# nuclia/nucliadb

Hardware: AMD Instinct MI355X
Metric: queries/sec + recall@10 (768-dim cosine k-NN, HNSW M=30 ef=30 ef_upper=4 build_ef_upper=4, k=10) (higher is better)
Workload: dtype f32

## Files before the change

### nucliadb_amd/csrc/hnsw_device.h

```cpp
#pragma once
#include "device_common.h"
#include "kernels.h"

namespace nidx {

#define NIDX_POOL_CAP 512
#define NIDX_VIS_EMPTY 0xffffffffu
#define NIDX_DEFER_CAP 256

struct NbBuf {
    uint32_t addr[64];
    float ab[64];
    float xx[64];
};
struct SearchShared {
    uint64_t pool[NIDX_POOL_CAP];
    NbBuf nb[2];
    uint32_t eps[256];
    int ctrl[12];
};

template <int NJ>
struct QueryRegs {
    float4 qv[NJ];
    float qq;
    double sqrt_qq;
};

template <int NJ>
__device__ inline void load_query(QueryRegs<NJ> &q, const float *qrow, uint32_t dp, int lane, bool cosine) {
    float acc = 0.f;
#pragma unroll
    for (int j = 0; j < NJ; j++) {
        q.qv[j] = load_row_chunk(qrow, dp, j, lane);
        acc = fma4(q.qv[j], q.qv[j], acc);
    }
    q.qq = wave_butterfly_sum(acc);
    q.sqrt_qq = cosine ? sqrt((double)q.qq) : 0.0;
}

__device__ inline float score_from_sums(float ab, float xx, float qq, double sqrt_qq, bool cosine) {
    if (!cosine) return ab;
    double dab = (double)ab, dxx = (double)xx;
    double dist;
    if (dxx == 0.0 && (double)qq == 0.0) dist = 0.0;
    else if (dab == 0.0) dist = 1.0;
    else {
        double d = 1.0 - dab / (sqrt(dxx) * sqrt_qq);
        dist = d > 0.0 ? d : 0.0;
    }
    return 1.0f - (float)dist;
}

__device__ inline uint32_t nidx_tid() {
    const uint32_t nw = blockDim.x >> 6;
    const uint32_t t = threadIdx.x + ((blockIdx.x % nw) << 6);
    return t >= blockDim.x ? t - blockDim.x : t;
}

__device__ inline void vis_clear(uint32_t *vis, uint32_t cap) {
    for (uint32_t i = nidx_tid(); i < cap; i += blockDim.x) vis[i] = NIDX_VIS_EMPTY;
}
__device__ inline bool vis_insert(uint32_t *vis, uint32_t log2cap, uint32_t v) {
    const uint32_t mask = (1u << log2cap) - 1u;
    uint32_t h = (v * 2654435761u) >> (32 - log2cap);
    for (;;) {
        uint32_t old = atomicCAS(&vis[h], NIDX_VIS_EMPTY, v);
        if (old == NIDX_VIS_EMPTY) return true;
        if (old == v) return false;
        h = (h + 1) & mask;
    }
}

__device__ inline bool vis_contains(const uint32_t *vis, uint32_t log2cap, uint32_t v) {
    const uint32_t mask = (1u << log2cap) - 1u;
    uint32_t h = (v * 2654435761u) >> (32 - log2cap);
    for (;;) {
        const uint32_t cur = vis[h];
        if (cur == NIDX_VIS_EMPTY) return false;
        if (cur == v) return true;
        h = (h + 1) & mask;
    }
}

__device__ inline uint64_t wave_max_u64(uint64_t v) { return wave_extreme_u64<true>(v); }
__device__ inline uint64_t wave_min_u64(uint64_t v) { return wave_extreme_u64<false>(v); }
__device__ inline uint64_t pool_peek(const uint64_t *pool, int pool_len, int lane) {
    uint64_t best = NIDX_EMPTY_KEY;
    for (int i = lane; i < pool_len; i += 64) {
        uint64_t v = pool[i];
        best = v > best ? v : best;
    }
    return wave_max_u64(best);
}
__device__ inline uint64_t pool_pop(uint64_t *pool, int &pool_len, int lane) {
    if (pool_len == 0) return NIDX_EMPTY_KEY;
    uint64_t best = NIDX_EMPTY_KEY;
    for (int i = lane; i < pool_len; i += 64) {
        uint64_t v = pool[i];
        best = v > best ? v : best;
    }
    best = wave_max_u64(best);
    int idx = 0x7fffffff;
    for (int i = lane; i < pool_len; i += 64)
        if (pool[i] == best && i < idx) idx = i;
    idx = wave_min_i32(idx);
    uint64_t last = pool[pool_len - 1];
    if (lane == 0) pool[idx] = last;
    pool_len--;
    return best;
}
__device__ inline void pool_prune(uint64_t *pool, int &pool_len, float ws, int lane) {
    int out = 0;
    for (int base = 0; base < pool_len; base += 64) {
        int i = base + lane;
        uint64_t v = i < pool_len ? pool[i] : NIDX_EMPTY_KEY;
        bool keep = i < pool_len && !(rank_key_score(v) < ws);
        unsigned long long m = __ballot(keep);
        int pos = out + __popcll(m & ((1ull << lane) - 1ull));
        if (keep) pool[pos] = v;
        out += __popcll(m);
    }
    pool_len = out;
}

template <int NL>
struct CandSet {
    uint64_t unexp[NL];
    __device__ inline void init() {
#pragma unroll
        for (int i = 0; i < NL; i++) unexp[i] = 0;
    }
    __device__ inline void insert(WaveTopK<NL> &res, uint64_t nk, int cap, int lane, uint64_t &out_key, bool &out_unexp) {
        uint64_t d = nk, dflag = 1;
#pragma unroll
        for (int i = 0; i < NL; i++) {
            if (d != NIDX_EMPTY_KEY) {
                const int pos = __popcll(__ballot(res.l[i].key > d));
                if (pos < 64) {
                    const uint64_t last = lane_bcast_u64(res.l[i].key, 63);
                    const uint64_t lastflag = unexp[i] >> 63;
                    const uint64_t up = wave_shr1_u64(res.l[i].key);
                    if (lane > pos) res.l[i].key = up;
                    if (lane == pos) res.l[i].key = d;
                    const uint64_t low = unexp[i] & ((1ull << pos) - 1ull);
                    const uint64_t high = pos < 63 ? ((unexp[i] >> pos) << (pos + 1)) : 0ull;
                    unexp[i] = low | (dflag << pos) | high;
                    d = last;
                    dflag = lastflag;
                }
            }
        }
        res.len++;
        out_key = NIDX_EMPTY_KEY;
        out_unexp = false;
        if (res.len > cap) {
            if (cap >= 64 * NL) {
                out_key = d;
                out_unexp = dflag != 0;
            }
#pragma unroll
            for (int i = 0; i < NL; i++)
                if ((cap >> 6) == i) {
                    out_key = lane_bcast_u64(res.l[i].key, cap & 63);
                    out_unexp = ((unexp[i] >> (cap & 63)) & 1ull) != 0;
                    if (lane == (cap & 63)) res.l[i].key = NIDX_EMPTY_KEY;
                    unexp[i] &= ~(1ull << (cap & 63));
                }
            res.len = cap;
        }
    }
    __device__ inline uint64_t peek(const WaveTopK<NL> &res) const {
#pragma unroll
        for (int i = 0; i < NL; i++)
            if (unexp[i]) return lane_bcast_u64(res.l[i].key, __builtin_ctzll(unexp[i]));
        return NIDX_EMPTY_KEY;
    }
    __device__ inline void peek2_except(const WaveTopK<NL> &res, uint64_t skip, uint64_t &a, uint64_t &b) const {
        a = b = NIDX_EMPTY_KEY;
        int found = 0;
#pragma unroll
        for (int i = 0; i < NL; i++) {
            uint64_t m = unexp[i];
            while (m && found < 2) {
                const uint64_t key = lane_bcast_u64(res.l[i].key, __builtin_ctzll(m));
                m &= m - 1ull;
                if (key == skip) continue;
                if (found == 0) a = key;
                else b = key;
                found++;
            }
        }
    }
    __device__ inline uint64_t pop(const WaveTopK<NL> &res) {
#pragma unroll
        for (int i = 0; i < NL; i++)
            if (unexp[i]) {
                const int r = __builtin_ctzll(unexp[i]);
                unexp[i] &= unexp[i] - 1ull;
                return lane_bcast_u64(res.l[i].key, r);
            }
        return NIDX_EMPTY_KEY;
    }
};

struct SearchCounters {
    uint32_t evals, expansions, visited, flags, edge_hits;
    uint64_t cyc_ctl, cyc_eval, cyc_ins;
};

template <int NJ, int EVR>
__device__ inline void eval_row_group(const SegDev &seg, const QueryRegs<NJ> &q, NbBuf &nb, int base, int n, bool cosine, int lane) {
    float4 row[EVR][NJ];
#pragma unroll
    for (int i = 0; i < EVR; i++) {
        if (base + i < n) {
            const float *r = seg.vectors + (size_t)nb.addr[base + i] * seg.dp;
#pragma unroll
            for (int j = 0; j < NJ; j++) row[i][j] = load_row_chunk(r, seg.dp, j, lane);
        } else {
#pragma unroll
            for (int j = 0; j < NJ; j++) row[i][j] = make_float4(0.f, 0.f, 0.f, 0.f);
        }
    }
    constexpr int NV_COS = 2 * EVR <= 2 ? 2 : (2 * EVR <= 4 ? 4 : 8);
    constexpr int NV_DOT = EVR <= 1 ? 1 : (EVR <= 2 ? 2 : 4);
    if (cosine) {
        float v[NV_COS];
#pragma unroll
        for (int i = 0; i < NV_COS; i++) v[i] = 0.f;
#pragma unroll
        for (int i = 0; i < EVR; i++) {
            float ab = 0.f, xx = 0.f;
#pragma unroll
            for (int j = 0; j < NJ; j++) {
                ab = fma4(row[i][j], q.qv[j], ab);
                xx = fma4(row[i][j], row[i][j], xx);
            }
            v[2 * i] = ab;
            v[2 * i + 1] = xx;
        }
        float r = QReduce<NV_COS>::run(v, lane);
        int which = QReduce<NV_COS>::query_of_lane(lane);
        if ((lane & QReduce<NV_COS>::group_mask()) == 0) {
            int i = which >> 1;
            if (i < EVR && base + i < n) {
                if ((which & 1) == 0) nb.ab[base + i] = r;
                else nb.xx[base + i] = r;
            }
        }
    } else {
        float v[NV_DOT];
#pragma unroll
        for (int i = 0; i < NV_DOT; i++) v[i] = 0.f;
#pragma unroll
        for (int i = 0; i < EVR; i++) {
            float ab = 0.f;
#pragma unroll
            for (int j = 0; j < NJ; j++) ab = fma4(row[i][j], q.qv[j], ab);
            v[i] = ab;
        }
        float r = QReduce<NV_DOT>::run(v, lane);
        int which = QReduce<NV_DOT>::query_of_lane(lane);
        if ((lane & QReduce<NV_DOT>::group_mask()) == 0 && which < EVR && base + which < n) nb.ab[base + which] = r;
    }
}

template <int NJ, int EVR>
__device__ inline void eval_neighbours(const SegDev &seg, const QueryRegs<NJ> &q, NbBuf &nb, int n, bool cosine) {
    const int lane = threadIdx.x & 63;
    const int wave = nidx_tid() >> 6;
    const int nwaves = blockDim.x >> 6;
    for (int base = wave * EVR; base < n; base += nwaves * EVR) eval_row_group<NJ, EVR>(seg, q, nb, base, n, cosine, lane);
}

template <int NJ, int EVR>
__device__ inline void eval_neighbours_dynamic(const SegDev &seg, const QueryRegs<NJ> &q, NbBuf &nb, int n, bool cosine, int *next_row) {
    const int lane = threadIdx.x & 63;
    for (;;) {
        int base = 0;
        if (lane == 0) base = atomicAdd(next_row, EVR);
        base = __builtin_amdgcn_readfirstlane(base);
        if (base >= n) break;
        eval_row_group<NJ, EVR>(seg, q, nb, base, n, cosine, lane);
    }
}

#define NIDX_CMD_EVAL 0
#define NIDX_CMD_CLEAR 1
#define NIDX_CMD_EXIT 2
__device__ inline void split_post(SearchShared &sh, int op, int p, int n, int lane) {
    if (lane == 0) {
        sh.ctrl[0] = op | (p << 2) | (n << 3);
        sh.ctrl[3] = 0;
    }
    lds_barrier();
}
__device__ inline void split_close() { lds_barrier(); }
__device__ inline uint32_t load_edge_word(const GraphDev &g, uint32_t node, int layer, int lane, uint32_t &deg) {
    uint32_t w = 0;
    if (layer == 0) {
        w = g.l0[(size_t)node * NIDX_L0_STRIDE + lane];
    } else {
        uint32_t base = g.upper_base[node];
        if (base != 0xffffffffu && lane < NIDX_UP_STRIDE) w = g.upper[((size_t)base + (layer - 1)) * NIDX_UP_STRIDE + lane];
    }
    deg = lane_bcast_u32(w, 0);
    return w;
}

template <int NJ, int EVR>
__device__ inline void split_worker_loop(const SegDev &seg, const QueryRegs<NJ> &q, SearchShared &sh, uint32_t *vis, uint32_t vis_cap, bool cosine) {
    for (;;) {
        lds_barrier();
        const int cmd = __builtin_amdgcn_readfirstlane(sh.ctrl[0]);
        const int op = cmd & 3;
        if (op == NIDX_CMD_EVAL) eval_neighbours_dynamic<NJ, EVR>(seg, q, sh.nb[(cmd >> 2) & 1], cmd >> 3, cosine, &sh.ctrl[3]);
        else if (op == NIDX_CMD_CLEAR) vis_clear(vis, vis_cap);
        lds_barrier();
        if (op == NIDX_CMD_EXIT) return;
    }
}

#define NIDX_PARK_SLOTS 4
#define NIDX_EPS_BARE 0
#define NIDX_EPS_PARKED 1
#define NIDX_EPS_CARRIED 2
template <int NJ, int EFL, int EVR, bool SPLIT = false>
__device__ inline void layer_search_block(const SegDev &seg, const GraphDev &g, int layer, int k,
                                          const QueryRegs<NJ> &q, SearchShared &sh, uint32_t *vis, uint32_t vis_log2,
                                          WaveTopK<EFL> &res, SearchCounters &st, int ep_mode = NIDX_EPS_BARE) {
    const int lane = threadIdx.x & 63;
    const bool ctl = SPLIT ? true : (nidx_tid() >> 6) == 0;
    const bool cosine = seg.similarity == 1;
    const uint32_t vis_cap = 1u << vis_log2;
    const bool carried = ep_mode == NIDX_EPS_CARRIED;
    int pool_len = 0;
    uint32_t vis_count = 0;

    if constexpr (SPLIT) {
        split_post(sh, NIDX_CMD_CLEAR, 0, 0, lane);
        vis_clear(vis, vis_cap);
        split_close();
    } else {
        vis_clear(vis, vis_cap);
        __syncthreads();
    }
    int n_new = sh.ctrl[2];
    if (n_new > k) k = n_new < 64 * EFL ? n_new : 64 * EFL;
    CandSet<EFL> cand;
    cand.init();
    const int n_eps = carried ? 0 : n_new;
    uint32_t ptag = 0xffffffffu, pbase = 0xffffffffu;
    uint32_t pt0 = 0xffffffffu, pt1 = 0xffffffffu, pt2 = 0xffffffffu, pt3 = 0xffffffffu;
    int n_park = 0;
    if (ep_mode != NIDX_EPS_BARE && n_new <= 64) n_park = n_new < NIDX_PARK_SLOTS ? n_new : NIDX_PARK_SLOTS;
    if (carried && ctl) {
#pragma unroll
        for (int i = 0; i < EFL; i++) {
            const int left = res.len - 64 * i;
            cand.unexp[i] = left >= 64 ? ~0ull : (left > 0 ? (1ull << left) - 1ull : 0ull);
            if (lane < left) vis_insert(vis, vis_log2, rank_key_addr(res.mine(i)));
        }
        st.evals += n_new;
        vis_count += n_new;
        if (lane < n_park) ptag = rank_key_addr(res.mine(0));
    }
    if (ctl && !carried) {
        res.init();
        if (lane < n_new) {
            uint32_t ep = sh.eps[lane];
            vis_insert(vis, vis_log2, ep);
            sh.nb[0].addr[lane] = ep;
            if (lane < n_park) ptag = ep;
        }
    }
    if (layer >= 1 && ptag != 0xffffffffu) pbase = g.upper_base[ptag];
    int ep_done = 0;
    while (ep_done < n_eps) {
        int chunk = n_eps - ep_done < 64 ? n_eps - ep_done : 64;
        if (ctl && ep_done > 0 && lane < chunk) {
            uint32_t ep = sh.eps[ep_done + lane];
            vis_insert(vis, vis_log2, ep);
            sh.nb[0].addr[lane] = ep;
        }
        if constexpr (SPLIT) {
            split_post(sh, NIDX_CMD_EVAL, 0, chunk, lane);
            split_close();
        } else {
            __syncthreads();
            eval_neighbours<NJ, EVR>(seg, q, sh.nb[0], chunk, cosine);
            __syncthreads();
        }
        if (ctl) {
            float s = lane < chunk ? score_from_sums(sh.nb[0].ab[lane], sh.nb[0].xx[lane], q.qq, q.sqrt_qq, cosine) : 0.f;
            uint32_t addr = sh.nb[0].addr[lane];
            for (int j = 0; j < chunk; j++) {
                uint64_t ek;
                bool eu;
                cand.insert(res, rank_key(lane_bcast_f32(s, j), lane_bcast_u32(addr, j)), 64 * EFL, lane, ek, eu);
            }
            st.evals += chunk;
            vis_count += chunk;
        }
        ep_done += chunk;
    }
    if (ctl && n_park > 0) {
        pt0 = lane_bcast_u32(ptag, 0);
        pt1 = lane_bcast_u32(ptag, 1);
        pt2 = lane_bcast_u32(ptag, 2);
        pt3 = lane_bcast_u32(ptag, 3);
        uint32_t w[NIDX_PARK_SLOTS];
#pragma unroll
        for (int r = 0; r < NIDX_PARK_SLOTS; r++) {
            w[r] = 0;
            if (r < n_park) {
                const uint32_t node = lane_bcast_u32(ptag, r), b = lane_bcast_u32(pbase, r);
                if (layer == 0) w[r] = g.l0[(size_t)node * NIDX_L0_STRIDE + lane];
                else if (b != 0xffffffffu && lane < NIDX_UP_STRIDE) w[r] = g.upper[((size_t)b + (layer - 1)) * NIDX_UP_STRIDE + lane];
            }
        }
#pragma unroll
        for (int r = 0; r < NIDX_PARK_SLOTS; r++)
            if (r < n_park) sh.eps[r * 64 + lane] = w[r];
    }

    uint32_t pw0 = 0, pw1 = 0, tg0 = 0xffffffffu, tg1 = 0xffffffffu;
    uint32_t edge_hits = 0;
    auto prepare = [&](uint64_t ck, NbBuf &dst) -> int {
        uint32_t deg;
        const uint32_t node = rank_key_addr(ck);
        uint32_t w;
        const int slot = node == pt0 ? 0 : (node == pt1 ? 1 : (node == pt2 ? 2 : (node == pt3 ? 3 : -1)));
        if (slot >= 0) {
            w = sh.eps[slot * 64 + lane];
            deg = lane_bcast_u32(w, 0);
            edge_hits++;
        } else if (node == tg0) {
            w = pw0;
            deg = lane_bcast_u32(w, 0);
            edge_hits++;
        } else if (node == tg1) {
            w = pw1;
            deg = lane_bcast_u32(w, 0);
            edge_hits++;
        } else {
            w = load_edge_word(g, node, layer, lane, deg);
        }
        const bool fresh = lane >= 1 && lane <= (int)deg && !vis_contains(vis, vis_log2, w);
        const unsigned long long m = __ballot(fresh);
        if (fresh) dst.addr[__popcll(m & ((1ull << lane) - 1ull))] = w;
        return __popcll(m);
    };
    int p = 0;
    uint64_t cur = NIDX_EMPTY_KEY;
    int cont = 0, n_cur_reg = 0;
    if (ctl) {
        const uint64_t t_a = clock64();
        int n0 = 0;
        cur = cand.pop(res);
        if (cur != NIDX_EMPTY_KEY && !(rank_key_score(cur) < res.worst_score())) {
            cont = 1;
            n0 = prepare(cur, sh.nb[0]);
        }
        n_cur_reg = n0;
        if (!SPLIT && lane == 0) {
            sh.ctrl[0] = cont;
            sh.ctrl[6] = n0;
            sh.ctrl[3] = 0;
        }
        st.cyc_ctl += clock64() - t_a;
    }
    if constexpr (SPLIT) {
        if (cont) {
            split_post(sh, NIDX_CMD_EVAL, 0, n_cur_reg, lane);
            split_close();
        }
    } else {
        lds_barrier();
        cont = sh.ctrl[0];
        if (cont) {
            eval_neighbours_dynamic<NJ, EVR>(seg, q, sh.nb[0], sh.ctrl[6], cosine, &sh.ctrl[3]);
            lds_barrier();
        }
    }
    if (cont) {
        for (;;) {
            NbBuf &nb_cur = sh.nb[p], &nb_next = sh.nb[p ^ 1];
            const int n_cur = SPLIT ? n_cur_reg : sh.ctrl[6 + p];
            float s = 0.f;
            uint32_t addr = 0;
            unsigned long long todo = 0;
            uint64_t nxt = NIDX_EMPTY_KEY;
            bool overflow = false;
            int n_next_reg = 0, redo_reg = 0;
            const uint64_t t_a = clock64();
            if (ctl) {
                const bool mine = lane < n_cur;
                addr = nb_cur.addr[lane];
                bool ins = mine && vis_insert(vis, vis_log2, addr);
                unsigned long long failed = __ballot(mine && !ins);
                while (failed) {
                    const int f = __ffsll((long long)failed) - 1;
                    failed &= failed - 1;
                    const unsigned long long same = __ballot(mine && addr == lane_bcast_u32(addr, f));
                    if ((same >> lane) & 1ull) ins = lane == __ffsll((long long)same) - 1;
                }
                todo = __ballot(ins);
                const int n_valid = __popcll(todo);
                st.expansions++;
                st.evals += n_valid;
                vis_count += n_valid;
                overflow = vis_count > vis_cap - vis_cap / 4;
                s = ins ? score_from_sums(nb_cur.ab[lane], nb_cur.xx[lane], q.qq, q.sqrt_qq, cosine) : 0.f;
                int n_next = 0;
                if (!overflow) {
                    const float ws = res.worst_score();
                    const bool adm = ins && (s > ws || res.len < k);
                    const uint64_t bn = wave_max_u64(adm ? rank_key(s, addr) : NIDX_EMPTY_KEY);
                    const uint64_t pm = cand.peek(res);
                    nxt = pm > bn ? pm : bn;
                    if (nxt == NIDX_EMPTY_KEY && pool_len > 0) nxt = pool_peek(sh.pool, pool_len, lane);
                    if (nxt != NIDX_EMPTY_KEY) n_next = prepare(nxt, nb_next);
                    if (layer == 0) {
                        uint64_t ka, kb;
                        cand.peek2_except(res, nxt, ka, kb);
                        uint32_t wa = ka != NIDX_EMPTY_KEY ? rank_key_addr(ka) : 0xffffffffu;
                        uint32_t wb = kb != NIDX_EMPTY_KEY ? rank_key_addr(kb) : 0xffffffffu;
                        if (wa == tg1 || wb == tg0) {
                            const uint32_t t = wa;
                            wa = wb;
                            wb = t;
                        }
                        if (wa != tg0) {
                            tg0 = wa;
                            if (wa != 0xffffffffu) pw0 = g.l0[(size_t)wa * NIDX_L0_STRIDE + lane];
                        }
                        if (wb != tg1) {
                            tg1 = wb;
                            if (wb != 0xffffffffu) pw1 = g.l0[(size_t)wb * NIDX_L0_STRIDE + lane];
                        }
                    }
                }
                n_next_reg = n_next;
                if (!SPLIT && lane == 0) {
                    sh.ctrl[5] = nxt != NIDX_EMPTY_KEY;
                    sh.ctrl[6 + (p ^ 1)] = n_next;
                    sh.ctrl[3] = 0;
                }
            }
            if constexpr (SPLIT) split_post(sh, NIDX_CMD_EVAL, p ^ 1, n_next_reg, lane);
            else lds_barrier();
            const uint64_t t_b = clock64();
            st.cyc_ctl += t_b - t_a;
            const bool has_next = SPLIT ? false : sh.ctrl[5] != 0;
            const int n_next = SPLIT ? n_next_reg : sh.ctrl[6 + (p ^ 1)];
            if (!ctl && has_next) eval_neighbours_dynamic<NJ, EVR>(seg, q, nb_next, n_next, cosine, &sh.ctrl[3]);
            if (ctl) {
                while (todo) {
                    float ws = res.worst_score();
                    if (res.len >= k) {
                        todo &= __ballot(s > ws);
                        if (!todo) break;
                    }
                    int j = __ffsll((long long)todo) - 1;
                    todo &= ~(1ull << j);
                    float sj = lane_bcast_f32(s, j);
                    if (sj > ws || res.len < k) {
                        uint64_t ek;
                        bool eu;
                        cand.insert(res, rank_key(sj, lane_bcast_u32(addr, j)), k, lane, ek, eu);
                        if (eu && ek != NIDX_EMPTY_KEY && !(rank_key_score(ek) < res.worst_score())) {
                            if (pool_len == NIDX_POOL_CAP) {
                                pool_prune(sh.pool, pool_len, res.worst_score(), lane);
                                if (pool_len == NIDX_POOL_CAP) {
                                    st.flags |= NIDX_FLAG_POOL_INEXACT;
                                    pool_len--;
                                }
                            }
                            if (lane == 0) sh.pool[pool_len] = ek;
                            pool_len++;
                        }
                    }
                }
                int redo = 0;
                cont = 0;
                if (overflow) {
                    st.flags |= NIDX_FLAG_VISITED_OVERFLOW;
                } else {
                    cur = cand.pop(res);
                    if (cur == NIDX_EMPTY_KEY && pool_len > 0) cur = pool_pop(sh.pool, pool_len, lane);
                    cont = cur != NIDX_EMPTY_KEY && !(rank_key_score(cur) < res.worst_score());
                    redo = cont && cur != nxt;
                }
                redo_reg = redo;
                if (!SPLIT && lane == 0) {
                    sh.ctrl[0] = cont;
                    sh.ctrl[4] = redo;
                }
                const uint64_t t_c = clock64();
                st.cyc_ins += t_c - t_b;
                if (has_next) eval_neighbours_dynamic<NJ, EVR>(seg, q, nb_next, n_next, cosine, &sh.ctrl[3]);
                st.cyc_eval += clock64() - t_c;
            }
            if constexpr (SPLIT) {
                split_close();
            } else {
                lds_barrier();
                cont = sh.ctrl[0];
                redo_reg = sh.ctrl[4];
            }
            if (!cont) break;
            n_cur_reg = n_next;
            if (redo_reg) {
                if (ctl) {
                    const int n1 = prepare(cur, nb_next);
                    n_cur_reg = n1;
                    if (!SPLIT && lane == 0) {
                        sh.ctrl[6 + (p ^ 1)] = n1;
                        sh.ctrl[3] = 0;
                    }
                }
                if constexpr (SPLIT) {
                    split_post(sh, NIDX_CMD_EVAL, p ^ 1, n_cur_reg, lane);
                    split_close();
                } else {
                    lds_barrier();
                    eval_neighbours_dynamic<NJ, EVR>(seg, q, nb_next, sh.ctrl[6 + (p ^ 1)], cosine, &sh.ctrl[3]);
                    lds_barrier();
                }
            }
            p ^= 1;
        }
    }
    st.edge_hits += edge_hits;
    st.visited = st.visited > vis_count ? st.visited : vis_count;
}

}
```

Before: 4.538 million.

## Statically partition split-worker neighbour rows and fetch command with first addresses

Split-mode worker waves stop claiming row groups through an LDS atomic counter and instead take a fixed strided share of rows by wave index. The command word and the first 16 neighbour addresses of both buffers are read in one LDS load per turn and spread with readlane. A specialised row-group evaluator handles partial groups by count and issues direct global float4 loads, with asm barriers steering values into scalar or vector registers. The intent is to remove the atomic traffic and the extra LDS round trips. The cost is possible load imbalance between waves and more code size from the per-count template instances.

```diff
diff --git a/nucliadb_amd/csrc/hnsw_device.h b/nucliadb_amd/csrc/hnsw_device.h
--- a/nucliadb_amd/csrc/hnsw_device.h
+++ b/nucliadb_amd/csrc/hnsw_device.h
@@ -1,4 +1,6 @@
 #pragma once
+#include <cstddef>
+
 #include "device_common.h"
 #include "kernels.h"
 
@@ -52,11 +54,12 @@
     return 1.0f - (float)dist;
 }
 
-__device__ inline uint32_t nidx_tid() {
+__device__ inline uint32_t nidx_tid_of(uint32_t tx) {
     const uint32_t nw = blockDim.x >> 6;
-    const uint32_t t = threadIdx.x + ((blockIdx.x % nw) << 6);
+    const uint32_t t = tx + ((blockIdx.x % nw) << 6);
     return t >= blockDim.x ? t - blockDim.x : t;
 }
+__device__ inline uint32_t nidx_tid() { return nidx_tid_of(threadIdx.x); }
 
 __device__ inline void vis_clear(uint32_t *vis, uint32_t cap) {
     for (uint32_t i = nidx_tid(); i < cap; i += blockDim.x) vis[i] = NIDX_VIS_EMPTY;
@@ -290,10 +293,7 @@
 #define NIDX_CMD_CLEAR 1
 #define NIDX_CMD_EXIT 2
 __device__ inline void split_post(SearchShared &sh, int op, int p, int n, int lane) {
-    if (lane == 0) {
-        sh.ctrl[0] = op | (p << 2) | (n << 3);
-        sh.ctrl[3] = 0;
-    }
+    if (lane == 0) sh.ctrl[0] = op | (p << 2) | (n << 3);
     lds_barrier();
 }
 __device__ inline void split_close() { lds_barrier(); }
@@ -309,14 +309,143 @@
     return w;
 }
 
+__device__ inline uint32_t opaque_u32(uint32_t v) {
+    asm volatile("" : "+v"(v));
+    return v;
+}
+__device__ inline uint32_t opaque_scalar_u32(uint32_t v) {
+    asm volatile("" : "+s"(v));
+    return v;
+}
+typedef float NativeF4 __attribute__((ext_vector_type(4)));
+__device__ inline float4 load_global_f4(uint64_t addr) {
+    const NativeF4 v = *(const NativeF4 __attribute__((address_space(1))) *)addr;
+    return make_float4(v.x, v.y, v.z, v.w);
+}
+
+template <int NJ, int EVR, int CNT>
+__device__ inline void split_row_group(const SegDev &seg, const QueryRegs<NJ> &q, NbBuf &nb, const uint32_t (&ra)[EVR], int base, bool cosine, uint32_t tx) {
+    static_assert(CNT >= 1 && CNT <= EVR, "a group holds 1 .. EVR rows");
+    constexpr int NWHOLE = NJ <= 4 ? NJ - 1 : 0;
+    float4 row[CNT][NJ];
+    uint64_t rb[CNT];
+#pragma unroll
+    for (int i = 0; i < CNT; i++) {
+        rb[i] = reinterpret_cast<uint64_t>(seg.vectors) + (((uint64_t)ra[i] * seg.dp) << 2);
+        asm volatile("" : "+s"(rb[i]));
+    }
+    const uint32_t t = opaque_u32(tx);
+    const uint32_t voff = (t & 63u) * 16u;
+    uint32_t vpart[NJ - NWHOLE];
+#pragma unroll
+    for (int j = NWHOLE; j < NJ; j++) vpart[j - NWHOLE] = (int)((t & 63u) * 4u) < (int)seg.dp - j * 256 ? voff + (uint32_t)j * 1024u : 0u;
+#pragma unroll
+    for (int i = 0; i < CNT; i++) {
+#pragma unroll
+        for (int j = 0; j < NJ; j++) {
+            if (j < NWHOLE) row[i][j] = load_global_f4(rb[i] + (uint64_t)voff + (uint64_t)(j * 1024));
+            else row[i][j] = load_global_f4(rb[i] + (uint64_t)vpart[j - NWHOLE]);
+        }
+    }
+    const int lane = opaque_u32(tx) & 63;
+    if (seg.dp != (uint32_t)NJ * 256u) {
+#pragma unroll
+        for (int j = NWHOLE; j < NJ; j++) {
+            if (!(lane * 4 < (int)seg.dp - j * 256)) {
+#pragma unroll
+                for (int i = 0; i < CNT; i++) row[i][j] = make_float4(0.f, 0.f, 0.f, 0.f);
+            }
+        }
+    }
+    constexpr int NV_COS = 2 * EVR <= 2 ? 2 : (2 * EVR <= 4 ? 4 : 8);
+    constexpr int NV_DOT = EVR <= 1 ? 1 : (EVR <= 2 ? 2 : 4);
+    if (cosine) {
+        float v[NV_COS];
+#pragma unroll
+        for (int i = 0; i < NV_COS; i++) v[i] = 0.f;
+#pragma unroll
+        for (int i = 0; i < CNT; i++) {
+            float ab = 0.f, xx = 0.f;
+#pragma unroll
+            for (int j = 0; j < NJ; j++) {
+                ab = fma4(row[i][j], q.qv[j], ab);
+                xx = fma4(row[i][j], row[i][j], xx);
+            }
+            v[2 * i] = ab;
+            v[2 * i + 1] = xx;
+        }
+        float r = QReduce<NV_COS>::run(v, lane);
+        int which = QReduce<NV_COS>::query_of_lane(lane);
+        static_assert(offsetof(NbBuf, xx) == offsetof(NbBuf, ab) + 64 * sizeof(float), "nb.xx follows nb.ab");
+        if ((lane & QReduce<NV_COS>::group_mask()) == 0 && (which >> 1) < CNT) (&nb.ab[0])[((which & 1) << 6) + base + (which >> 1)] = r;
+    } else {
+        float v[NV_DOT];
+#pragma unroll
+        for (int i = 0; i < NV_DOT; i++) v[i] = 0.f;
+#pragma unroll
+        for (int i = 0; i < CNT; i++) {
+            float ab = 0.f;
+#pragma unroll
+            for (int j = 0; j < NJ; j++) ab = fma4(row[i][j], q.qv[j], ab);
+            v[i] = ab;
+        }
+        float r = QReduce<NV_DOT>::run(v, lane);
+        int which = QReduce<NV_DOT>::query_of_lane(lane);
+        if ((lane & QReduce<NV_DOT>::group_mask()) == 0 && which < CNT) nb.ab[base + which] = r;
+    }
+}
+
+template <int NJ, int EVR>
+__device__ inline void split_row_group_n(const SegDev &seg, const QueryRegs<NJ> &q, NbBuf &nb, const uint32_t (&ra)[EVR], int base, int cnt, bool cosine, uint32_t tx) {
+    if constexpr (EVR >= 2) {
+        if (cnt == 1) return split_row_group<NJ, EVR, 1>(seg, q, nb, ra, base, cosine, tx);
+    }
+    if constexpr (EVR >= 3) {
+        if (cnt == 2) return split_row_group<NJ, EVR, 2>(seg, q, nb, ra, base, cosine, tx);
+    }
+    if constexpr (EVR >= 4) {
+        if (cnt == 3) return split_row_group<NJ, EVR, 3>(seg, q, nb, ra, base, cosine, tx);
+    }
+    split_row_group<NJ, EVR, EVR>(seg, q, nb, ra, base, cosine, tx);
+}
+
 template <int NJ, int EVR>
 __device__ inline void split_worker_loop(const SegDev &seg, const QueryRegs<NJ> &q, SearchShared &sh, uint32_t *vis, uint32_t vis_cap, bool cosine) {
+    static_assert(EVR <= 4, "a first group must lie in the 16 addresses per buffer that the turn's one read fetches");
+    const int w = __builtin_amdgcn_readfirstlane((int)(nidx_tid() >> 6)) - 1, nw = (int)(blockDim.x >> 6) - 1;
+    const uint32_t tx = threadIdx.x;
+    const uint32_t *words = sh.nb[0].addr;
+    constexpr uint32_t NB_WORDS = sizeof(NbBuf) / 4, CMD_WORD = (offsetof(SearchShared, ctrl) - offsetof(SearchShared, nb)) / 4;
     for (;;) {
+        const uint32_t t = opaque_u32(tx);
+        const uint32_t head_at = (t & 63u) < 32u ? ((t >> 4) & 1u) * opaque_scalar_u32(NB_WORDS) + (t & 15u) : opaque_u32(CMD_WORD);
         lds_barrier();
-        const int cmd = __builtin_amdgcn_readfirstlane(sh.ctrl[0]);
+        const uint32_t head = words[head_at];
+        const int cmd = __builtin_amdgcn_readlane((int)head, 32);
         const int op = cmd & 3;
-        if (op == NIDX_CMD_EVAL) eval_neighbours_dynamic<NJ, EVR>(seg, q, sh.nb[(cmd >> 2) & 1], cmd >> 3, cosine, &sh.ctrl[3]);
-        else if (op == NIDX_CMD_CLEAR) vis_clear(vis, vis_cap);
+        if (op == NIDX_CMD_EVAL) {
+            const int p = (cmd >> 2) & 1, n = cmd >> 3;
+            NbBuf &nb = sh.nb[p];
+            const int stride = nw * EVR;
+            int base = w * EVR;
+            if (base < n) {
+                uint32_t ra[EVR];
+#pragma unroll
+                for (int i = 0; i < EVR; i++) ra[i] = (uint32_t)__builtin_amdgcn_readlane((int)head, p * 16 + base + i);
+                for (;;) {
+                    split_row_group_n<NJ, EVR>(seg, q, nb, ra, base, n - base < EVR ? n - base : EVR, cosine, tx);
+                    base += stride;
+                    if (base >= n) break;
+                    const int r = base + (int)(opaque_u32(tx) & 3u);
+                    const uint32_t more = nb.addr[r < 63 ? r : 63];
+#pragma unroll
+                    for (int i = 0; i < EVR; i++) ra[i] = (uint32_t)__builtin_amdgcn_readlane((int)more, i);
+                }
+            }
+        } else if (op == NIDX_CMD_CLEAR) {
+            const uint32_t empty = opaque_u32(NIDX_VIS_EMPTY);
+            for (uint32_t i = nidx_tid_of(t); i < vis_cap; i += blockDim.x) vis[i] = empty;
+        }
         lds_barrier();
         if (op == NIDX_CMD_EXIT) return;
     }
```

New measurement: 4.716 million (median of 6 runs). 1.04x the previous value.
